# grasingerm/polymer-stats

Hardware: AMD Instinct MI355X
Metric: MC monomer-updates/sec (whole node) at n=100 (higher is better)
Workload: dtype f64

## Files before the change

polymer_stats_amd/csrc/pstat_api.hip:

```cpp
#include <hip/hip_runtime.h>

#include <cmath>
#include <cstdarg>
#include <cstdio>
#include <cstdlib>
#include <cstring>
#include <memory>
#include <new>
#include <vector>

#include "../../include/pstat.h"
#include "pstat_cluster_common.h"
#include "pstat_device.h"

using namespace pstat;

namespace {

thread_local char g_err[512] = "";

int fail(int code, const char *fmt, ...) {
  va_list ap;
  va_start(ap, fmt);
  vsnprintf(g_err, sizeof g_err, fmt, ap);
// ... 357 lines not shown
  p->cutoff_radius = 7.5;
}

int pstat_create(const pstat_params *cases, int32_t ncases, void *stream, pstat_handle **out) {
  if (!cases || !out) return fail(PSTAT_ERR_INVALID_ARG, "null argument");
  *out = nullptr;
  int rc = validate(cases, ncases);
  if (rc) return rc;
  int ndev = pstat_device_count();
  if (ndev < 1) return fail(PSTAT_ERR_NO_DEVICE, "no HIP device is visible (this library has no CPU path)");
  if (cases[0].device < 0 || cases[0].device >= ndev)
    return fail(PSTAT_ERR_NO_DEVICE, "device %d out of range (have %d)", cases[0].device, ndev);

  pstat_handle *h = new (std::nothrow) pstat_handle;
  if (!h) return fail(PSTAT_ERR_NOMEM, "host allocation failed");
  try {
  h->base = cases[0];
  h->ncases = ncases;
  h->device = cases[0].device;
  h->elem = cases[0].precision == PSTAT_F64 ? 8 : (cases[0].precision == PSTAT_Q16 ? 2 : 4);
  for (int i = 0; i < ncases; ++i) {
    const pstat_params &p = cases[i];
    h->cases.push_back({p.E0, p.K1, p.K2, p.mu, p.kT, p.Fz, p.Fx, p.b, p.seed, p.chain_id0,
                        p.bend_mod, p.bend_angle, p.cluster_prob, p.cutoff_radius});
    h->kT0.push_back(p.kT);
  }
  bool any_fx = false;
  for (auto &c : h->cases) any_fx = any_fx || c.Fx != 0.0;
  h->ov = read_overrides();
  h->cfg = {h->base.precision, h->base.chain_type, h->base.energy_type, h->base.do_flips ? 1 : 0,
            h->base.umbrella ? 1 : 0, any_fx ? 1 : 0, 0, h->base.rng, h->base.move_set};
  const Home home = h->cfg.home = choose_home(h->cfg, h->base.n, h->base.num_chains, ncases, h->ov);

  int lanes = (home == SweepLds || home == ClusterLds) ? choose_lanes(h->base.precision, h->base.n, h->base.energy_type) : 64;
  if (lanes == 0) {
    delete h;
    return fail(PSTAT_ERR_UNSUPPORTED, "num-monomers = %lld does not fit the 160 KiB LDS of a CU",
                (long long)cases[0].n);
  }
  SweepArgs &A = h->args;
  A.n = h->base.n;
  A.chains_per_case = h->base.num_chains;
  A.blocks_per_case = (h->base.num_chains + lanes - 1) / lanes;
  A.nblocks = A.blocks_per_case * ncases;
  A.nsteps = 0; A.step0 = 0;
  A.steps_per_adjust = h->base.steps_per_adjust;
  A.adj_lb = h->base.adj_lb; A.adj_ub = h->base.adj_ub; A.adj_scale = h->base.adj_scale;
  A.lanes = lanes;
  A.adaptive = (h->base.adj_scale != 1.0 && h->base.steps_per_adjust > 0) ? 1 : 0;
  A.ncases = ncases; A.seg_len = 0; A.nseg = 1; A.max_spins = 1 << 22;
  A.lds_rows = 0; A.packed = 0; A.pad_ = 0;
  A.wide_eps = (h->base.precision == PSTAT_F64 && h->base.uniform_bits != 23) ? 1 : 0;
  if (home == SweepMem) {
    int rows = 160 * 1024 / 4 / (64 * 16) - 1;
    if (h->ov.f64_lds_rows >= 0 && h->ov.f64_lds_rows <= rows) rows = h->ov.f64_lds_rows;
    A.lds_rows = (int32_t)(h->base.n < rows ? h->base.n : rows);
  }

#define CREATE_TRY(expr)            \
  do {                              \
    int _rc = (expr);               \
    if (_rc) { pstat_destroy(h); return _rc; } \
  } while (0)
#define CREATE_HIP(expr)                                                                   \
  do {                                                                                     \
    hipError_t _e = (expr);                                                                \
    if (_e != hipSuccess) {                                                                \
      pstat_destroy(h);                                                                    \
      return fail(PSTAT_ERR_HIP, "%s failed: %s", #expr, hipGetErrorString(_e));           \
    }                                                                                      \
  } while (0)

  CREATE_HIP(hipSetDevice(h->device));
  hipDeviceProp_t prop;
  if (chain_per_lane(home)) {
    CREATE_HIP(hipGetDeviceProperties(&prop, h->device));
    Shape pick = shape(h->cfg, A, false, false, prop.multiProcessorCount, h->ov.lanes);
    if (ncases > 1) {
      const Shape pk = shape(h->cfg, A, true, pick.cost >= 4.0 || h->ov.pack == 1, prop.multiProcessorCount, h->ov.lanes);
      if (h->ov.pack >= 0 ? h->ov.pack == 1 : pk.cost < 0.95 * pick.cost) {
        pick = pk;
        h->cfg.packed = 1;
        A.packed = 1;
      }
    }
    A.lanes = pick.lanes;
    A.blocks_per_case = (h->base.num_chains + pick.lanes - 1) / pick.lanes;
// ... 526 lines not shown
```

polymer_stats_amd/csrc/pstat_device.h:

```cpp
#pragma once

#include <hip/hip_runtime.h>
#include <stdint.h>

namespace pstat {

enum { OBS_R1 = 0, OBS_R2, OBS_R3, OBS_P1, OBS_P2, OBS_P3, OBS_U, OBS_USUM,
       OBS_C2,
       OBS_PSI,
       NOBS_STATE };
enum { S_R1 = 0, S_R2, S_R3, S_R1SQ, S_R2SQ, S_R3SQ, S_P1, S_P2, S_P3, S_P1SQ, S_P2SQ, S_P3SQ,
       S_U, S_USQ, NSUMS_BASE, S_C2 = NSUMS_BASE, S_PSI, NSUMS };

struct DevState {
  void *ang;
  void *ang_tmp;
  uint32_t *rng;
  double *stepsz;
  int64_t *win;
  int64_t *nacc_total;
  double *obs;
  double *sums;
  double *wnorm;
  double *lag;
// ... 198 lines not shown
struct LaunchCfg {
  int precision, chain_type, energy_type, do_flips, umbrella, has_fx;
  int lag;
  int rng;
  int move_set;
  Home home;
  int packed;
};
hipError_t launch_init(const LaunchCfg &cfg, const SweepArgs &a, const DevState &s,
                       const CaseConst *cases, double phi_step, double theta_step,
                       const InitOpts &io, hipStream_t stream);
hipError_t launch_reset_sampler(const DevState &s, double phi_step, double theta_step, hipStream_t stream);
hipError_t launch_cluster(const LaunchCfg &cfg, const SweepArgs &a, const DevState &s,
                          const CaseConst *cases, int *queue, unsigned grid, hipStream_t stream);
hipError_t cluster_kernel_info(const LaunchCfg &cfg, const SweepArgs &a, int *lds_bytes,
                               int *blocks_per_cu, const char **name);
hipError_t launch_cluster_gm(const LaunchCfg &cfg, const SweepArgs &a, const DevState &s,
                             const CaseConst *cases, int *queue, unsigned grid, hipStream_t stream);
hipError_t cluster_gm_kernel_info(const LaunchCfg &cfg, const SweepArgs &a, int *lds_bytes,
                                  int *blocks_per_cu, const char **name);
size_t cluster_gm_work_bytes(const LaunchCfg &cfg, const SweepArgs &a);
hipError_t launch_sweep(const LaunchCfg &cfg, const SweepArgs &a, const DevState &s,
                        const CaseConst *cases, int *queue, unsigned grid, hipStream_t stream);
size_t sweep_queue_ints(const SweepArgs &a);
hipError_t launch_reinit(const LaunchCfg &cfg, const SweepArgs &a, const DevState &s,
                         const CaseConst *cases, int force_init, hipStream_t stream);
template <typename R> __host__ __device__ inline bool not_finite(R x) { return !__builtin_isfinite(x); }
hipError_t launch_reduce(const DevState &s, int64_t c0, int64_t c1, int64_t steps_recorded,
                         int umbrella, const CaseConst *cases, int64_t chains_per_case, int64_t n,
                         double *partial, double *out, hipStream_t stream);
size_t reduce_scratch_doubles();
hipError_t sweep_kernel_info(const LaunchCfg &cfg, const SweepArgs &a, int *lds_bytes,
                             int *blocks_per_cu, const char **name);
int choose_lanes(int precision, int64_t n, int energy_type);
hipError_t launch_interacting(const LaunchCfg &cfg, const SweepArgs &a, const DevState &s,
                              const CaseConst *cases, int reinit_mode, hipStream_t stream);
hipError_t launch_cluster_wave(const LaunchCfg &cfg, const SweepArgs &a, const DevState &s, const CaseConst *cases,
                               hipStream_t stream);
hipError_t cluster_wave_kernel_info(const LaunchCfg &cfg, int64_t n, int *blocks_per_cu, const char **name);
hipError_t launch_cluster_cw(const LaunchCfg &cfg, const SweepArgs &a, const DevState &s, const CaseConst *cases,
                             hipStream_t stream);
hipError_t cluster_cw_kernel_info(const LaunchCfg &cfg, int64_t n, int *blocks_per_cu, const char **name);
hipError_t interacting_kernel_info(const LaunchCfg &cfg, int64_t n, int *blocks_per_cu, const char **name);

}
```

polymer_stats_amd/csrc/pstat_kernels.hip:

```cpp
#include "pstat_device.h"

#include <hip/hip_runtime.h>
#include <math.h>
#include <type_traits>

#include "../../include/pstat.h"
#include "pstat_math.h"

#ifndef PSTAT_GM_DEPTH
#define PSTAT_GM_DEPTH 2
#endif
#ifndef PSTAT_GI_DEPTH
#define PSTAT_GI_DEPTH 1
#endif
#ifndef PSTAT_GI_CC
#define PSTAT_GI_CC 1
#endif
#ifndef PSTAT_UNROLL_ISING
#define PSTAT_UNROLL_ISING 16
#endif
#ifndef PSTAT_UNROLL
#define PSTAT_UNROLL 16
#endif

// ... 84 lines not shown
  d.w0 = g.next();
  d.idx = __umulhi(d.w0, n);
  d.cell = __umul24(d.idx, row_bytes) + lane_bytes;
  d.wphi = g.next();
  d.wflip = 0;
  if constexpr (RARE) {
    if (flips) d.wflip = g.next();
  }
  d.wth = g.next();
  d.weps = g.next();
  return d;
}

struct SweepRare {
  int flips;
  int lag;
  int umb;
};

template <typename R, typename G, int CT, int EN, bool FX, bool RARE, int ST>
__device__ __forceinline__ void run_segment(const SweepArgs &A, const DevState &S, const CaseConst &cc,
                                            const SweepRare rare, unsigned char *smem, const int lane,
                                            const int64_t c, int64_t step, int64_t remaining, const int blk) {
  using R2 = typename Vec2<R>::type;
  using AG = Ang<R>;
  constexpr bool Q = ST == 1;
  constexpr bool GM = ST == 2;
  static_assert(!Q || sizeof(R) == 4, "the lattice state runs on f32 arithmetic");
  static_assert(!GM || sizeof(R) == 8, "global-memory state: f64");
  constexpr bool GI = GM && EN == PSTAT_ISING;
  constexpr int DEPTH = GI ? PSTAT_GI_DEPTH : PSTAT_GM_DEPTH;
  using Cell = typename std::conditional<Q, uint32_t, R2>::type;
  const int lanes = GM ? 64 : A.lanes;
  unsigned char *const cells = GM ? reinterpret_cast<unsigned char *>(S.work) + (size_t)blk * (size_t)A.n * 64 * sizeof(Cell) : smem;
  Cell *ang = reinterpret_cast<Cell *>(cells);
  const int64_t C = S.C;
  const int n = (int)A.n;

  const R Fz = (R)cc.Fz, Fx = (R)cc.Fx, b = (R)cc.b, kT = (R)cc.kT;
  const R a_or_mu = (CT == PSTAT_DIELECTRIC) ? (R)((cc.K1 - cc.K2) * cc.E0) : (R)cc.mu;
  const R k2e = (R)(cc.K2 * cc.E0);
  const R mhalfE0 = (R)(-0.5 * cc.E0);
  const R hb = (R)(-cc.b / 2);
  const R ising_scale = cc.b == 0.0 ? (R)__builtin_nan("") : (R)(0.0795774715459476679 / fabs(cc.b * cc.b * cc.b / 8));
  const R nbeta_log2e = (R)(-1.4426950408889634 / cc.kT);
  const double ninv_kT = -1.0 / cc.kT;
  (void)ninv_kT;
  (void)Fx; (void)kT; (void)hb; (void)nbeta_log2e; (void)ising_scale;

  R maxphi = 0;
  (void)maxphi;
  if constexpr (Q) {
    const uint16_t *gth = (const uint16_t *)S.ang, *gph = (const uint16_t *)S.ang + (int64_t)n * C;
#pragma unroll 8
    for (int i = 0; i < n; ++i)
      ang[i * lanes + lane] = (uint32_t)gth[(int64_t)i * C + c] | ((uint32_t)gph[(int64_t)i * C + c] << 16);
  } else {
    const R *gth = (const R *)S.ang, *gph = (const R *)S.ang + (int64_t)n * C;
#pragma unroll 8
    for (int i = 0; i < n; ++i) {
      R2 v;
      v.x = gth[(int64_t)i * C + c];
      v.y = gph[(int64_t)i * C + c];
      if constexpr (sizeof(R) == 8) maxphi = fmax(maxphi, fabs(v.y));
      if (GM && i < A.lds_rows) reinterpret_cast<Cell *>(smem)[i * lanes + lane] = v;
      else if constexpr (GM) *reinterpret_cast<Cell *>(cells + ((EN == PSTAT_ISING && PSTAT_GI_CC) ? (uint32_t)lane * (uint32_t)n * (uint32_t)sizeof(Cell) + (uint32_t)i * (uint32_t)sizeof(Cell)
                                                                                                          : (uint32_t)(i * lanes + lane) * (uint32_t)sizeof(Cell))) = v;
      else ang[i * lanes + lane] = v;
    }
  }
  constexpr double th_unit = Q ? 3.14159265358979323846 / 65536.0 : AG::unit;
  constexpr double ph_unit = Q ? 6.28318530717958647692 / 65536.0 : AG::unit;
  G g;
  g.load(S.rng + c, C);
  double phistep_d = S.stepsz[0 * C + c], thstep_d = S.stepsz[1 * C + c];
  R phistep = (R)(phistep_d / ph_unit), thstep = (R)(thstep_d / th_unit);
  int64_t nacc_off = S.win[0 * C + c], natt_off = S.win[1 * C + c];
  int nacc_seg = 0, steps_seg = 0;
  int nnan_seg = 0;
  R O[8];
  O[0] = (R)S.obs[OBS_R1 * C + c]; O[1] = (R)S.obs[OBS_R2 * C + c]; O[2] = (R)S.obs[OBS_R3 * C + c];
  O[3] = (R)S.obs[OBS_P1 * C + c]; O[4] = (R)S.obs[OBS_P2 * C + c]; O[5] = (R)S.obs[OBS_P3 * C + c];
  O[6] = (R)S.obs[OBS_U * C + c]; O[7] = 0;
  R usum = (R)S.obs[OBS_USUM * C + c];
  R lag = RARE ? (R)S.lag[c] : (R)0;
  const bool umb = RARE && rare.umb;
  const R wscale = umb ? (R)((0.2 + 0.8 * exp(-(cc.Fx * cc.Fx + cc.Fz * cc.Fz) / cc.kT)) / cc.kT) : (R)0;
  R uref = umb ? (R)S.uref[c] : (R)0;
  bool regauged = false;
  double wnorm = umb ? S.wnorm[c] : 0.0;
  double sums[NSUMS_BASE];
#pragma unroll
  for (int q = 0; q < NSUMS_BASE; ++q) sums[q] = S.sums[q * C + c];

  const int64_t spa = A.steps_per_adjust;
  int64_t to_adj = A.adaptive ? spa - (step % spa) : 0;
  constexpr int FLUSH = 128;
  const bool flips = RARE && rare.flips;

  using P = typename V2<R>::type;
  const uint32_t row_bytes = (uint32_t)lanes * (uint32_t)sizeof(Cell), lane_bytes = (uint32_t)lane * (uint32_t)sizeof(Cell);
  auto slot = [&](uint32_t off) __attribute__((always_inline)) -> Cell & { return *reinterpret_cast<Cell *>(cells + off); };
  constexpr bool CC = GI && PSTAT_GI_CC;
  const uint32_t chain_g = (uint32_t)lane * (uint32_t)n * (uint32_t)sizeof(Cell);
  auto gofs = [&](const uint32_t idx) __attribute__((always_inline)) -> uint32_t {
    return CC ? chain_g + idx * (uint32_t)sizeof(Cell) : idx * row_bytes + lane_bytes;
  };
  typedef int v4i __attribute__((ext_vector_type(4)));
  struct RowG { Cell l; v4i g; };
  struct RowG3 { RowG c, lo, hi; };
  using Row = typename std::conditional<GI, RowG3, typename std::conditional<GM, RowG, Cell>::type>::type;
  const uint32_t nL = GM ? (uint32_t)A.lds_rows : 0u;
  const uint32_t trash = nL * row_bytes + lane_bytes;
  __amdgpu_buffer_rsrc_t rsrc = __builtin_amdgcn_make_buffer_rsrc(GM ? (void *)cells : (void *)nullptr, 0,
                                                                  GM ? (int)((uint32_t)n * row_bytes) : 0, 0x00020000);
  auto rdcell = [&](const uint32_t idx, const uint32_t cell) __attribute__((always_inline)) -> RowG {
    const bool inL = idx < nL;
    RowG r;
    r.l = *reinterpret_cast<Cell *>(smem + (inL ? cell : trash));
    r.g = __builtin_amdgcn_raw_buffer_load_b128(rsrc, inL ? 0xFFFFFFFFu : gofs(idx), 0, 0);
    return r;
  };
  auto resolve = [&](const RowG &r, const uint32_t idx, const uint32_t cell, const Cell &f1, const uint32_t at1,
                     const Cell &f2, const uint32_t at2, const Cell &f3, const uint32_t at3) __attribute__((always_inline)) -> Cell {
    if constexpr (GM) {
      typedef double v2dd __attribute__((ext_vector_type(2)));
      const v2dd gv = __builtin_bit_cast(v2dd, r.g);
      const bool inL = idx < nL;
      Cell a;
      a.x = inL ? r.l.x : gv.x; a.y = inL ? r.l.y : gv.y;
      if constexpr (DEPTH == 3) {
        const bool s3 = at3 == cell;
        a.x = s3 ? f3.x : a.x; a.y = s3 ? f3.y : a.y;
      }
      if constexpr (DEPTH >= 2) {
        const bool s2 = at2 == cell;
        a.x = s2 ? f2.x : a.x; a.y = s2 ? f2.y : a.y;
      }
      const bool s1 = at1 == cell;
      a.x = s1 ? f1.x : a.x; a.y = s1 ? f1.y : a.y;
      return a;
    } else {
      return r.l;
    }
  };
  auto rdrow = [&](const Draw &d) __attribute__((always_inline)) -> Row {
    if constexpr (GI) {
      const bool hasLo = d.idx > 0, hasHi = d.idx + 1 < (uint32_t)n;
      RowG3 r;
      r.c = rdcell(d.idx, d.cell);
      r.lo = rdcell(hasLo ? d.idx - 1 : d.idx, hasLo ? d.cell - row_bytes : d.cell);
      r.hi = rdcell(hasHi ? d.idx + 1 : d.idx, hasHi ? d.cell + row_bytes : d.cell);
      return r;
    } else if constexpr (GM) {
      return rdcell(d.idx, d.cell);
    } else {
      return slot(d.cell);
    }
  };
  auto wr = [&](const Draw &d, const Cell v, const bool ok) __attribute__((always_inline)) {
    if constexpr (GM) {
      const bool inL = d.idx < nL;
      *reinterpret_cast<Cell *>(smem + ((ok && inL) ? d.cell : trash)) = v;
      typedef double v2dd __attribute__((ext_vector_type(2)));
      const v2dd vv = {v.x, v.y};
      __builtin_amdgcn_raw_buffer_store_b128(__builtin_bit_cast(v4i, vv), rsrc, (ok && !inL) ? gofs(d.idx) : 0xFFFFFFFFu, 0, 0);
    } else {
      slot(d.cell) = v;
    }
  };
  Draw dA = draw_step<RARE>(g, (uint32_t)n, flips, row_bytes, lane_bytes), dB = dA;
  Row aA = rdrow(dA), aB = aA;
  Draw dC = dA;
  Row aC = aA;
  Draw dD = dA;
  Row aD = aA;
  Cell fw1_cell{}, fw2_cell{}, fw3_cell{};
  uint32_t fw1_at = ~0u, fw2_at = ~0u, fw3_at = ~0u;
  (void)dC; (void)aC; (void)dD; (void)aD; (void)fw1_cell; (void)fw2_cell; (void)fw3_cell; (void)fw1_at; (void)fw2_at; (void)fw3_at;
  if constexpr (GM && DEPTH >= 2) {
    if (remaining > 1) {
      dB = draw_step<RARE>(g, (uint32_t)n, flips, row_bytes, lane_bytes);
      aB = rdrow(dB);
    }
    if constexpr (DEPTH == 3) {
      if (remaining > 2) {
        dC = draw_step<RARE>(g, (uint32_t)n, flips, row_bytes, lane_bytes);
        aC = rdrow(dC);
      }
    }
  }
  R phistep3 = 3 * phistep, thstep3 = 3 * thstep;
  (void)phistep3; (void)thstep3;
  P stepv = {thstep, phistep}, step3v = {thstep3, phistep3};
  (void)stepv; (void)step3v;
  int left = (int)remaining;
// ... 80 lines not shown
        if constexpr (RARE) {
          if (flips && (d.wflip >> 31)) k0 = 65535u - k0;
        }
        const int k1 = (int)k0 + q16_disp(thstep, sym11<R>(d.wth));
        const uint32_t j1 = (j0 + (uint32_t)q16_disp(phistep, sym11<R>(d.wphi))) & 0xFFFFu;
        inside = (uint32_t)k1 < 65536u;
        const uint32_t k1c = (uint32_t)min(max(k1, 0), 65535);
        th1 = q16_theta_turns(k1c);
        ph1 = q16_phi_turns(j1);
        cell1 = k1c | (j1 << 16);
      } else {
        th0 = a0.x; ph0 = a0.y;
        R flip = 0;
        if constexpr (RARE) {
          if (flips && (d.wflip >> 31)) flip = AG::theta_max - 2 * th0;
        }
        if constexpr (sizeof(R) == 8) {
          auto rounded = [](R v) __attribute__((always_inline)) -> R { asm volatile("" : "+v"(v)); return v; };
          const R dphi = rounded(phistep * rounded(sym11<R>(d.wphi)));
          R dth = rounded(thstep * rounded(sym11<R>(d.wth)));
          if constexpr (RARE) dth = rounded(flip + dth);
          ph1 = AG::wrap(ph0 + dphi);
          th1 = fmin(AG::theta_max, fmax((R)0, th0 + dth));
        } else {
          R base = th0;
          if constexpr (RARE) base = th0 + flip;
          const P basev = {base, ph0}, fv = {bits24(d.wth), bits24(d.wphi)};
          const P raw = pfma(stepv, fv, basev - step3v);
          th1 = fmin(AG::theta_max, fmax((R)0, raw.x));
          ph1 = AG::wrap(raw.y);
        }
      }
      R st0, ct0, sp0, cp0, st1, ct1, sp1, cp1;
      AG::sc_theta(th0, &st0, &ct0);
      AG::sc_theta(th1, &st1, &ct1);
      AG::template sc_phi<FOLD>(ph0, &sp0, &cp0);
      AG::template sc_phi<FOLD>(ph1, &sp1, &cp1);
      P dNxy, dMxy, D;
      R dpair = 0;
      if constexpr (EN == PSTAT_ISING && sizeof(R) == 4) {
        const P S01 = {st0, st1}, X01 = P{cp0, cp1} * S01, Y01 = P{sp0, sp1} * S01, C01 = {ct0, ct1};
        P MX01, MY01, MZ01;
        if constexpr (CT == PSTAT_DIELECTRIC) {
          const P q01 = C01 * P{a_or_mu, a_or_mu};
          MX01 = q01 * X01; MY01 = q01 * Y01;
          MZ01 = pfma(q01, C01, P{k2e, k2e});
        } else {
          const P mus = {a_or_mu, a_or_mu};
          MX01 = mus * X01; MY01 = mus * Y01; MZ01 = mus * C01;
        }
        dNxy = P{X01.y - X01.x, Y01.y - Y01.x};
        dMxy = P{MX01.y - MX01.x, MY01.y - MY01.x};
        D = P{C01.y - C01.x, MZ01.y - MZ01.x};
        P e01 = {0, 0};
        const P m3 = {-3.0f, -3.0f};
#pragma unroll
        for (int side = -1; side <= 1; side += 2) {
          const int j = (int)d.idx + side;
          if (j >= 0 && j < n) {
            const Cell aj = ang[j * lanes + lane];
            R thj, phj;
            if constexpr (Q) { thj = q16_theta_turns(aj & 0xFFFFu); phj = q16_phi_turns(aj >> 16); }
            else { thj = aj.x; phj = aj.y; }
            R sj, cj, spj, cpj, mjx, mjy, mjz;
            AG::sc(thj, &sj, &cj);
            AG::sc(phj, &spj, &cpj);
            const R njx = cpj * sj, njy = spj * sj, njz = cj;
            dipole<R, CT>(a_or_mu, k2e, njx, njy, njz, mjx, mjy, mjz);
            const P rx = X01 + P{njx, njx}, ry = Y01 + P{njy, njy}, rz = C01 + P{njz, njz};
            const P jx = {mjx, mjx}, jy = {mjy, mjy}, jz = {mjz, mjz};
// ... 5 lines not shown
            const P mjr = pfma(jz, rz, pfma(jy, ry, jx * rx));
            const P num = pfma(m3 * ir2, mir * mjr, mimj);
            e01 = pfma(num, ir2 * ir, e01);
          }
        }
        dpair = (e01.y - e01.x) * ising_scale;
      } else {
        const P cs0 = {cp0, sp0}, cs1 = {cp1, sp1};
        const P s0s = {st0, st0}, s1s = {st1, st1};
        const P Nxy0 = cs0 * s0s, Nxy1 = cs1 * s1s;
        P Mxy0, Mxy1;
        R mz0, mz1;
        if constexpr (CT == PSTAT_DIELECTRIC) {
          const R q0 = a_or_mu * ct0, q1 = a_or_mu * ct1;
          const P q0s = {q0, q0}, q1s = {q1, q1};
          Mxy0 = q0s * Nxy0; Mxy1 = q1s * Nxy1;
          mz0 = q0 * ct0 + k2e; mz1 = q1 * ct1 + k2e;
        } else {
          const P mus = {a_or_mu, a_or_mu};
          Mxy0 = mus * Nxy0; Mxy1 = mus * Nxy1;
          mz0 = a_or_mu * ct0; mz1 = a_or_mu * ct1;
        }
        dNxy = Nxy1 - Nxy0; dMxy = Mxy1 - Mxy0;
        const P Z0 = {ct0, mz0}, Z1 = {ct1, mz1};
        D = Z1 - Z0;

        if constexpr (GI) {
          R e0 = 0, e1 = 0;
#pragma unroll
          for (int side = 0; side < 2; ++side) {
            const Cell aj = side ? aHi : aLo;
            const bool has = side ? d.idx + 1 < (uint32_t)n : d.idx > 0;
            R sj, cj, spj, cpj, mjx, mjy, mjz;
            AG::sc_theta(aj.x, &sj, &cj);
            AG::template sc_phi<FOLD>(aj.y, &spj, &cpj);
            const R njx = cpj * sj, njy = spj * sj, njz = cj;
            dipole<R, CT>(a_or_mu, k2e, njx, njy, njz, mjx, mjy, mjz);
            const R t0 = pair_term_fast(hb * (Nxy0.x + njx), hb * (Nxy0.y + njy), hb * (ct0 + njz),
                                        Mxy0.x, Mxy0.y, mz0, mjx, mjy, mjz);
            const R t1 = pair_term_fast(hb * (Nxy1.x + njx), hb * (Nxy1.y + njy), hb * (ct1 + njz),
                                        Mxy1.x, Mxy1.y, mz1, mjx, mjy, mjz);
            e0 += has ? t0 : (R)0; e1 += has ? t1 : (R)0;
          }
          dpair = e1 - e0;
        } else if constexpr (EN == PSTAT_ISING) {
          R e0 = 0, e1 = 0;
  #pragma unroll
          for (int side = -1; side <= 1; side += 2) {
            const int j = (int)d.idx + side;
            if (j >= 0 && j < n) {
              const Cell aj = ang[j * lanes + lane];
              R thj, phj;
              if constexpr (Q) { thj = q16_theta_turns(aj & 0xFFFFu); phj = q16_phi_turns(aj >> 16); }
              else { thj = aj.x; phj = aj.y; }
              R sj, cj, spj, cpj, mjx, mjy, mjz;
              AG::sc(thj, &sj, &cj);
              AG::sc(phj, &spj, &cpj);
              const R njx = cpj * sj, njy = spj * sj, njz = cj;
              dipole<R, CT>(a_or_mu, k2e, njx, njy, njz, mjx, mjy, mjz);
              e0 += pair_term_fast(hb * (Nxy0.x + njx), hb * (Nxy0.y + njy), hb * (ct0 + njz),
                                   Mxy0.x, Mxy0.y, mz0, mjx, mjy, mjz);
              e1 += pair_term_fast(hb * (Nxy1.x + njx), hb * (Nxy1.y + njy), hb * (ct1 + njz),
                                   Mxy1.x, Mxy1.y, mz1, mjx, mjy, mjz);
            }
          }
          dpair = e1 - e0;
        }
      }
// ... 171 lines not shown
          phistep_d = fmin(K<double>::pi, phistep_d * A.adj_scale);
          thstep_d = fmin(K<double>::half_pi, thstep_d * A.adj_scale);
        } else if (ratio < A.adj_lb) {
          nacc_off = -nacc_seg; natt_off = -steps_seg;
          phistep_d /= A.adj_scale;
          thstep_d /= A.adj_scale;
        }
        phistep = (R)(phistep_d / ph_unit); thstep = (R)(thstep_d / th_unit);
        phistep3 = 3 * phistep; thstep3 = 3 * thstep;
        stepv = P{thstep, phistep}; step3v = P{thstep3, phistep3};
      }
    }
  }
  };
  if constexpr (sizeof(R) == 8) {
    const bool can_reach = !((double)maxphi + 3.1416 * (double)remaining < PSTAT_PHI_FOLD);
    if (__builtin_amdgcn_ballot_w64(can_reach) != 0) run_steps(std::true_type{});
    else run_steps(std::false_type{});
  } else {
    run_steps(std::false_type{});
  }

  if constexpr (Q) {
    uint16_t *gth = (uint16_t *)S.ang, *gph = (uint16_t *)S.ang + (int64_t)n * C;
    for (int i = 0; i < n; ++i) {
      const uint32_t v = ang[i * lanes + lane];
      gth[(int64_t)i * C + c] = (uint16_t)(v & 0xFFFFu);
      gph[(int64_t)i * C + c] = (uint16_t)(v >> 16);
    }
  } else {
    R *gth = (R *)S.ang, *gph = (R *)S.ang + (int64_t)n * C;
    for (int i = 0; i < n; ++i) {
      R2 v;
      if (GM && i < A.lds_rows) v = reinterpret_cast<Cell *>(smem)[i * lanes + lane];
      else if constexpr (GM) v = *reinterpret_cast<Cell *>(cells + gofs((uint32_t)i));
      else v = ang[i * lanes + lane];
      gth[(int64_t)i * C + c] = v.x;
      gph[(int64_t)i * C + c] = v.y;
    }
  }
  g.store(S.rng + c, C);
  S.stepsz[0 * C + c] = phistep_d; S.stepsz[1 * C + c] = thstep_d;
  S.win[0 * C + c] = nacc_off + nacc_seg; S.win[1 * C + c] = natt_off + steps_seg;
  S.nacc_total[c] += nacc_seg;
  if constexpr (EN == PSTAT_ISING) S.nanrej[c] += nnan_seg;
  const R unit_r = sizeof(R) == 4 ? b : (R)1;
  S.obs[OBS_R1 * C + c] = unit_r * Orxy.x; S.obs[OBS_R2 * C + c] = unit_r * Orxy.y; S.obs[OBS_R3 * C + c] = unit_r * Oz.x;
  S.obs[OBS_P1 * C + c] = Opxy.x; S.obs[OBS_P2 * C + c] = Opxy.y; S.obs[OBS_P3 * C + c] = Oz.y;
  S.obs[OBS_U * C + c] = OU;
  if constexpr (RARE) S.obs[OBS_USUM * C + c] = usum;
  if constexpr (RARE) {
    S.lag[c] = lag;
    if (umb) S.wnorm[c] = wnorm;
    if (regauged) S.uref[c] = (double)uref;
  }
#pragma unroll
  for (int q = 0; q < NSUMS_BASE; ++q) S.sums[q * C + c] = sums[q];
}

template <typename R, typename G, int CT, int EN, bool FX, bool RARE, int ST, bool PACKED = false>
__global__ __launch_bounds__(64) void sweep_kernel(SweepArgs A, DevState S,
                                                   const CaseConst *__restrict__ cases,
                                                   SweepRare rare, int *__restrict__ queue) {
  extern __shared__ __attribute__((aligned(16))) unsigned char smem[];
  const int lane = threadIdx.x;
  run_job_queue<PACKED>(A, queue, lane, [&](const CaseConst &cc, int64_t chain, int64_t first, int64_t len, int blk) {
    run_segment<R, G, CT, EN, FX, RARE, ST>(A, S, cc, rare, smem, lane, chain, first, len, blk);
  }, cases);
}

#ifndef PSTAT_PART

constexpr int RED_BLOCKS = 256;
constexpr int RED_THREADS = 256;
constexpr int NQ = 19;
constexpr int NX = 2;
constexpr int NP = 2 * NQ + NX;

__device__ __forceinline__ double wave_sum(double v) {
#pragma unroll
  for (int off = 32; off > 0; off >>= 1) v += __shfl_down(v, off, 64);
  return v;
}

__global__ __launch_bounds__(RED_THREADS) void reduce_stage1(DevState S, int64_t c0, int64_t c1,
                                                             int64_t steps, int umbrella,
                                                             const CaseConst *__restrict__ cases,
                                                             int64_t chains_per_case, int64_t n,
                                                             double *__restrict__ partial) {
  __shared__ double red[RED_THREADS / 64][NP];
  double m1[NQ], m2[NQ], mx[NX] = {0, 0};
#pragma unroll
  for (int q = 0; q < NQ; ++q) { m1[q] = 0; m2[q] = 0; }
  const int64_t C = S.C;
  for (int64_t c = c0 + (int64_t)blockIdx.x * RED_THREADS + threadIdx.x; c < c1;
       c += (int64_t)RED_BLOCKS * RED_THREADS) {
    const double norm = umbrella ? S.wnorm[c] : (double)steps;
    const double inv = norm != 0.0 ? 1.0 / norm : 0.0;
// ... 142 lines not shown
  if (cfg.has_fx) return rare ? pick_state<G, CT, EN, true, true>() : pick_state<G, CT, EN, true, false>();
  return rare ? pick_state<G, CT, EN, false, true>() : pick_state<G, CT, EN, false, false>();
}
template <typename G>
static SweepFn pick_model(const LaunchCfg &cfg) {
  const bool ising = cfg.energy_type == PSTAT_ISING;
  if (cfg.chain_type == PSTAT_DIELECTRIC)
    return ising ? pick_flags<G, PSTAT_DIELECTRIC, PSTAT_ISING>(cfg)
                 : pick_flags<G, PSTAT_DIELECTRIC, PSTAT_NONINTERACTING>(cfg);
  return ising ? pick_flags<G, PSTAT_POLAR, PSTAT_ISING>(cfg)
               : pick_flags<G, PSTAT_POLAR, PSTAT_NONINTERACTING>(cfg);
}
#if PSTAT_PART == 4
SweepFn pick_sweep_f64g(const LaunchCfg &cfg) {
#elif PSTAT_PART == 3
SweepFn pick_sweep_f64(const LaunchCfg &cfg) {
#elif PSTAT_PART == 2
SweepFn pick_sweep_q16(const LaunchCfg &cfg) {
#else
SweepFn pick_sweep_f32(const LaunchCfg &cfg) {
#endif
  return cfg.rng == PSTAT_RNG_XOSHIRO128PP ? pick_model<Xoshiro128pp>(cfg) : pick_model<Mwc64x>(cfg);
}

#else

SweepFn pick_sweep_f32(const LaunchCfg &cfg);
SweepFn pick_sweep_q16(const LaunchCfg &cfg);
SweepFn pick_sweep_f64(const LaunchCfg &cfg);
SweepFn pick_sweep_f64g(const LaunchCfg &cfg);

static int cell_bytes(int precision) { return precision == PSTAT_F64 ? 16 : (precision == PSTAT_Q16 ? 4 : 8); }

int choose_lanes(int precision, int64_t n, int energy_type) {
  (void)energy_type;
  const int64_t per_lane = n * cell_bytes(precision);
  const int64_t budget = 160 * 1024;
  for (int lanes = 64; lanes >= 8; lanes >>= 1)
    if (per_lane * lanes <= budget) return lanes;
  return 0;
}

static SweepFn pick_sweep(const LaunchCfg &cfg) {
  if (cfg.home == SweepMem) return pick_sweep_f64g(cfg);
  return cfg.precision == PSTAT_F64 ? pick_sweep_f64(cfg)
       : (cfg.precision == PSTAT_Q16 ? pick_sweep_q16(cfg) : pick_sweep_f32(cfg));
}

static int sweep_lds_bytes(const LaunchCfg &cfg, const SweepArgs &a) {
  if (cfg.home == SweepMem) return (a.lds_rows + 1) * 64 * 16;
  return (int)(a.n * a.lanes * cell_bytes(cfg.precision));
}

hipError_t sweep_kernel_info(const LaunchCfg &cfg, const SweepArgs &a, int *lds_bytes,
                             int *blocks_per_cu, const char **name) {
  SweepFn fn = pick_sweep(cfg);
  const int lds = sweep_lds_bytes(cfg, a);
  hipError_t e = hipFuncSetAttribute((const void *)fn, hipFuncAttributeMaxDynamicSharedMemorySize, lds);
  if (e != hipSuccess) return e;
  int nb = 0;
  e = hipOccupancyMaxActiveBlocksPerMultiprocessor(&nb, (const void *)fn, 64, lds);
  if (e != hipSuccess) return e;
  if (lds_bytes) *lds_bytes = lds;
  if (blocks_per_cu) *blocks_per_cu = nb;
  if (name) *name = cfg.precision == PSTAT_F64 ? (cfg.home == SweepMem ? (cfg.packed ? "sweep_kernel<double, state in L2> [packed cases]" : "sweep_kernel<double, state in L2>")
                                                                   : (cfg.packed ? "sweep_kernel<double> [packed cases]" : "sweep_kernel<double>"))
                 : (cfg.precision == PSTAT_Q16 ? (cfg.packed ? "sweep_kernel<float, q16 state> [packed cases]" : "sweep_kernel<float, q16 state>")
                                               : (cfg.packed ? "sweep_kernel<float> [packed cases]" : "sweep_kernel<float>"));
  return hipSuccess;
}

size_t sweep_queue_ints(const SweepArgs &a) { return 2 + (size_t)a.nblocks; }

hipError_t launch_sweep(const LaunchCfg &cfg, const SweepArgs &a, const DevState &s,
                        const CaseConst *cases, int *queue, unsigned grid, hipStream_t stream) {
  SweepFn fn = pick_sweep(cfg);
  const int lds = sweep_lds_bytes(cfg, a);
  hipError_t e = hipFuncSetAttribute((const void *)fn, hipFuncAttributeMaxDynamicSharedMemorySize, lds);
  if (e != hipSuccess) return e;
  e = hipMemsetAsync(queue + 1, 0, sizeof(int) * (sweep_queue_ints(a) - 1), stream);
  if (e != hipSuccess) return e;
  SweepRare rare{cfg.do_flips, cfg.lag, cfg.umbrella};
  hipLaunchKernelGGL(fn, dim3(grid), dim3(64), lds, stream, a, s, cases, rare, queue);
  return hipGetLastError();
// ... 71 lines not shown
```

polymer_stats_amd/csrc/pstat_math.h:

```cpp
#pragma once

#include <hip/hip_runtime.h>
#include <math.h>
#include <stdint.h>

#include "../../include/pstat.h"

namespace pstat {


template <typename R> struct Vec2;
template <> struct Vec2<float> { using type = float2; };
template <> struct Vec2<double> { using type = double2; };

template <typename R> struct K;
template <> struct K<double> {
  static constexpr double pi = 3.14159265358979323846;
  static constexpr double half_pi = 1.57079632679489661923;
};

__device__ __forceinline__ double exp_f64(const double x) {
  const double k = rint(x * 1.44269504088896338700e+00);
  const double hi = __builtin_fma(-k, 6.93147180369123816490e-01, x);
  const double r = __builtin_fma(-k, 1.90821492927058770002e-10, hi);
// ... 246 lines not shown
    }
  }
  const double k = rint(x * 6.36619772367581382433e-01);
  const double r = __builtin_fma(-k, 6.12323399573676603587e-17, __builtin_fma(-k, 1.57079632679489655800e+00, x));
  const double z = r * r;
  const double S1 = -1.66666666666666324348e-01, S2 = 8.33333333332248946124e-03, S3 = -1.98412698298579493134e-04,
               S4 = 2.75573137070700676789e-06, S5 = -2.50507602534068634195e-08, S6 = 1.58969099521155010221e-10;
  const double C1 = 4.16666666666666019037e-02, C2 = -1.38888888888741095749e-03, C3 = 2.48015872894767294178e-05,
               C4 = -2.75573143513906633035e-07, C5 = 2.08757232129817482790e-09, C6 = -1.13596475577881948265e-11;
  const double ps = __builtin_fma(z, __builtin_fma(z, __builtin_fma(z, __builtin_fma(z, __builtin_fma(z, S6, S5), S4), S3), S2), S1);
  const double pc = __builtin_fma(z, __builtin_fma(z, __builtin_fma(z, __builtin_fma(z, __builtin_fma(z, C6, C5), C4), C3), C2), C1);
#ifndef PSTAT_THETA_GENERIC_TAIL
  if constexpr (BOUNDED) {
    const double ks = __builtin_fma(r * z, ps, r);
    const double kc = __builtin_fma(z, __builtin_fma(z, pc, -0.5), 1.0);
    const bool one = k == 1.0, two = k == 2.0;
    const double cq = two ? -kc : kc;
    *s = one ? kc : __builtin_fabs(ks);
    *c = one ? -ks : cq;
    return;
  }
#endif
  const uint32_t q = (uint32_t)(int)k;
  const uint32_t odd = q << 31;
  const uint32_t m_kc = (q >> 1) << 31;
  const uint32_t m_ks = m_kc ^ odd;
  const double rs = __hiloint2double((int)(__double2hiint(r) ^ m_ks), __double2loint(r));
  const double ks = __builtin_fma(rs * z, ps, rs);
  const double kc0 = __builtin_fma(z, __builtin_fma(z, pc, -0.5), 1.0);
  const double kc = __hiloint2double((int)(__double2hiint(kc0) ^ m_kc), __double2loint(kc0));
  const bool swap = (int)odd < 0;
  *s = swap ? kc : ks;
  *c = swap ? ks : kc;
}

__device__ __forceinline__ float acos_r(float x) {
  const float a = fabsf(x);
  float p = -0.0012624911f;
  p = __builtin_fmaf(p, a, 0.0066700901f);
  p = __builtin_fmaf(p, a, -0.0170881256f);
  p = __builtin_fmaf(p, a, 0.0308918810f);
  p = __builtin_fmaf(p, a, -0.0501743046f);
  p = __builtin_fmaf(p, a, 0.0889789874f);
  p = __builtin_fmaf(p, a, -0.2145988016f);
  p = __builtin_fmaf(p, a, 1.5707963050f);
  const float r = __builtin_amdgcn_sqrtf(fmaxf(1.0f - a, 0.0f)) * p;
  return x < 0.0f ? 3.14159265358979f - r : r;
}
__device__ __forceinline__ double acos_r(double x) {
  const double a = fabs(x);
  const bool big = a >= 0.5;
  const double z = big ? __builtin_fma(a, -0.5, 0.5) : a * a;
  double p = 2.87578513674215663354e-02;
  p = __builtin_fma(p, z, -1.48518870712472036977e-02);
  p = __builtin_fma(p, z, 1.74008794426940213707e-02);
  p = __builtin_fma(p, z, 5.45750671864035814818e-03);
  p = __builtin_fma(p, z, 1.03228143501857792808e-02);
  p = __builtin_fma(p, z, 1.14791774151849056834e-02);
  p = __builtin_fma(p, z, 1.39712129735529329289e-02);
  p = __builtin_fma(p, z, 1.73523927208699725588e-02);
  p = __builtin_fma(p, z, 2.23721729421498885526e-02);
  p = __builtin_fma(p, z, 3.03819441385312465076e-02);
  p = __builtin_fma(p, z, 4.46428571463554288434e-02);
  p = __builtin_fma(p, z, 7.49999999999843292020e-02);
  p = __builtin_fma(p, z, 1.66666666666666685170e-01);
  const double zp = z * p;
  const double y = __builtin_amdgcn_rsq(z);
  const double s0 = z * y, h0 = 0.5 * y;
  const double r = __builtin_fma(-s0, h0, 0.5);
  const double s1 = __builtin_fma(s0, r, s0), h1 = __builtin_fma(h0, r, h0);
  double sq = __builtin_fma(__builtin_fma(-s1, s1, z), h1, s1);
  sq = z == 0.0 ? 0.0 : sq;
  const double t = big ? sq : x;
  const double as = __builtin_fma(t, zp, t);
  const double small = 1.57079632679489661923 - as;
  const double two = as + as;
  const double bigv = x < 0.0 ? 3.14159265358979323846 - two : two;
  return big ? bigv : small;
}

template <typename R> struct Ang;
template <> struct Ang<double> {
  static constexpr double theta_max = 3.14159265358979323846;
  static constexpr double unit = 1.0;
  static __device__ __forceinline__ void sc(double x, double *s, double *c) { sincos_f64(x, s, c); }
  static __device__ __forceinline__ void sc_theta(double x, double *s, double *c) { sincos_fast_f64<true>(x, s, c); }
  template <bool FOLD = true>
  static __device__ __forceinline__ void sc_phi(double x, double *s, double *c) { sincos_fast_f64<false, FOLD>(x, s, c); }
  static __device__ __forceinline__ double wrap(double x) { return x; }
};
template <> struct Ang<float> {
  static constexpr float theta_max = 0.5f;
  static constexpr double unit = 6.28318530717958647692;
  static __device__ __forceinline__ void sc(float x, float *s, float *c) {
    *s = __builtin_amdgcn_sinf(x);
    *c = __builtin_amdgcn_cosf(x);
  }
  static __device__ __forceinline__ void sc_theta(float x, float *s, float *c) { sc(x, s, c); }
  template <bool FOLD = true>
  static __device__ __forceinline__ void sc_phi(float x, float *s, float *c) { sc(x, s, c); }
  static __device__ __forceinline__ float wrap(float x) { return __builtin_amdgcn_fractf(x); }
};


}
```

Before: 102.8 billion.

## Use LDS-resident 64-entry sincos table for f64 angle evaluation in sweep kernel

Replaces the polynomial f64 sincos in the sweep kernel with a table-driven scheme. The argument is reduced to a multiple of pi/32 plus a small remainder, the sin/cos of the multiple is looked up from a 1 KiB table held in LDS, and a short polynomial on the remainder finishes the result. The kernel fills the table at startup, and the LDS budgets (lanes, rows) are shrunk to make room for it. The aim is to cut FP64 instruction count per proposal, at the cost of extra LDS reads, possible bank conflicts, slightly less LDS for cells, and different rounding behaviour.

```diff
diff --git a/polymer_stats_amd/csrc/pstat_api.hip b/polymer_stats_amd/csrc/pstat_api.hip
--- a/polymer_stats_amd/csrc/pstat_api.hip
+++ b/polymer_stats_amd/csrc/pstat_api.hip
@@ -413,7 +413,8 @@
             h->base.umbrella ? 1 : 0, any_fx ? 1 : 0, 0, h->base.rng, h->base.move_set};
   const Home home = h->cfg.home = choose_home(h->cfg, h->base.n, h->base.num_chains, ncases, h->ov);
 
-  int lanes = (home == SweepLds || home == ClusterLds) ? choose_lanes(h->base.precision, h->base.n, h->base.energy_type) : 64;
+  const int tab_bytes = (home == SweepLds && h->base.precision == PSTAT_F64) ? PSTAT_SINCOS_TAB_BYTES : 0;
+  int lanes = (home == SweepLds || home == ClusterLds) ? choose_lanes(h->base.precision, h->base.n, h->base.energy_type, tab_bytes) : 64;
   if (lanes == 0) {
     delete h;
     return fail(PSTAT_ERR_UNSUPPORTED, "num-monomers = %lld does not fit the 160 KiB LDS of a CU",
@@ -433,7 +434,7 @@
   A.lds_rows = 0; A.packed = 0; A.pad_ = 0;
   A.wide_eps = (h->base.precision == PSTAT_F64 && h->base.uniform_bits != 23) ? 1 : 0;
   if (home == SweepMem) {
-    int rows = 160 * 1024 / 4 / (64 * 16) - 1;
+    int rows = 160 * 1024 / 4 / (64 * 16) - 2;
     if (h->ov.f64_lds_rows >= 0 && h->ov.f64_lds_rows <= rows) rows = h->ov.f64_lds_rows;
     A.lds_rows = (int32_t)(h->base.n < rows ? h->base.n : rows);
   }
diff --git a/polymer_stats_amd/csrc/pstat_device.h b/polymer_stats_amd/csrc/pstat_device.h
--- a/polymer_stats_amd/csrc/pstat_device.h
+++ b/polymer_stats_amd/csrc/pstat_device.h
@@ -254,7 +254,8 @@
 size_t reduce_scratch_doubles();
 hipError_t sweep_kernel_info(const LaunchCfg &cfg, const SweepArgs &a, int *lds_bytes,
                              int *blocks_per_cu, const char **name);
-int choose_lanes(int precision, int64_t n, int energy_type);
+#define PSTAT_SINCOS_TAB_BYTES 1024
+int choose_lanes(int precision, int64_t n, int energy_type, int table_bytes);
 hipError_t launch_interacting(const LaunchCfg &cfg, const SweepArgs &a, const DevState &s,
                               const CaseConst *cases, int reinit_mode, hipStream_t stream);
 hipError_t launch_cluster_wave(const LaunchCfg &cfg, const SweepArgs &a, const DevState &s, const CaseConst *cases,
diff --git a/polymer_stats_amd/csrc/pstat_kernels.hip b/polymer_stats_amd/csrc/pstat_kernels.hip
--- a/polymer_stats_amd/csrc/pstat_kernels.hip
+++ b/polymer_stats_amd/csrc/pstat_kernels.hip
@@ -140,7 +140,10 @@
   constexpr int DEPTH = GI ? PSTAT_GI_DEPTH : PSTAT_GM_DEPTH;
   using Cell = typename std::conditional<Q, uint32_t, R2>::type;
   const int lanes = GM ? 64 : A.lanes;
-  unsigned char *const cells = GM ? reinterpret_cast<unsigned char *>(S.work) + (size_t)blk * (size_t)A.n * 64 * sizeof(Cell) : smem;
+  const unsigned char *const tab = smem;
+  unsigned char *const lds = smem + (sizeof(R) == 8 ? PSTAT_SINCOS_TAB_BYTES : 0);
+  (void)tab;
+  unsigned char *const cells = GM ? reinterpret_cast<unsigned char *>(S.work) + (size_t)blk * (size_t)A.n * 64 * sizeof(Cell) : lds;
   Cell *ang = reinterpret_cast<Cell *>(cells);
   const int64_t C = S.C;
   const int n = (int)A.n;
@@ -171,7 +174,7 @@
       v.x = gth[(int64_t)i * C + c];
       v.y = gph[(int64_t)i * C + c];
       if constexpr (sizeof(R) == 8) maxphi = fmax(maxphi, fabs(v.y));
-      if (GM && i < A.lds_rows) reinterpret_cast<Cell *>(smem)[i * lanes + lane] = v;
+      if (GM && i < A.lds_rows) reinterpret_cast<Cell *>(lds)[i * lanes + lane] = v;
       else if constexpr (GM) *reinterpret_cast<Cell *>(cells + ((EN == PSTAT_ISING && PSTAT_GI_CC) ? (uint32_t)lane * (uint32_t)n * (uint32_t)sizeof(Cell) + (uint32_t)i * (uint32_t)sizeof(Cell)
                                                                                                           : (uint32_t)(i * lanes + lane) * (uint32_t)sizeof(Cell))) = v;
       else ang[i * lanes + lane] = v;
@@ -225,7 +228,7 @@
   auto rdcell = [&](const uint32_t idx, const uint32_t cell) __attribute__((always_inline)) -> RowG {
     const bool inL = idx < nL;
     RowG r;
-    r.l = *reinterpret_cast<Cell *>(smem + (inL ? cell : trash));
+    r.l = *reinterpret_cast<Cell *>(lds + (inL ? cell : trash));
     r.g = __builtin_amdgcn_raw_buffer_load_b128(rsrc, inL ? 0xFFFFFFFFu : gofs(idx), 0, 0);
     return r;
   };
@@ -269,7 +272,7 @@
   auto wr = [&](const Draw &d, const Cell v, const bool ok) __attribute__((always_inline)) {
     if constexpr (GM) {
       const bool inL = d.idx < nL;
-      *reinterpret_cast<Cell *>(smem + ((ok && inL) ? d.cell : trash)) = v;
+      *reinterpret_cast<Cell *>(lds + ((ok && inL) ? d.cell : trash)) = v;
       typedef double v2dd __attribute__((ext_vector_type(2)));
       const v2dd vv = {v.x, v.y};
       __builtin_amdgcn_raw_buffer_store_b128(__builtin_bit_cast(v4i, vv), rsrc, (ok && !inL) ? gofs(d.idx) : 0xFFFFFFFFu, 0, 0);
@@ -416,10 +419,21 @@
         }
       }
       R st0, ct0, sp0, cp0, st1, ct1, sp1, cp1;
-      AG::sc_theta(th0, &st0, &ct0);
-      AG::sc_theta(th1, &st1, &ct1);
-      AG::template sc_phi<FOLD>(ph0, &sp0, &cp0);
-      AG::template sc_phi<FOLD>(ph1, &sp1, &cp1);
+      if constexpr (sizeof(R) == 8) {
+        const SincosArg r0 = sincos_tab_reduce<false>(th0), r1 = sincos_tab_reduce<false>(th1);
+        const SincosArg r2 = sincos_tab_reduce<FOLD>(ph0), r3 = sincos_tab_reduce<FOLD>(ph1);
+        const double2 e0 = *reinterpret_cast<const double2 *>(tab + r0.at), e1 = *reinterpret_cast<const double2 *>(tab + r1.at);
+        const double2 e2 = *reinterpret_cast<const double2 *>(tab + r2.at), e3 = *reinterpret_cast<const double2 *>(tab + r3.at);
+        sincos_tab_finish(r0.r, e0, &st0, &ct0);
+        sincos_tab_finish(r1.r, e1, &st1, &ct1);
+        sincos_tab_finish(r2.r, e2, &sp0, &cp0);
+        sincos_tab_finish(r3.r, e3, &sp1, &cp1);
+      } else {
+        AG::sc_theta(th0, &st0, &ct0);
+        AG::sc_theta(th1, &st1, &ct1);
+        AG::template sc_phi<FOLD>(ph0, &sp0, &cp0);
+        AG::template sc_phi<FOLD>(ph1, &sp1, &cp1);
+      }
       P dNxy, dMxy, D;
       R dpair = 0;
       if constexpr (EN == PSTAT_ISING && sizeof(R) == 4) {
@@ -491,8 +505,8 @@
             const Cell aj = side ? aHi : aLo;
             const bool has = side ? d.idx + 1 < (uint32_t)n : d.idx > 0;
             R sj, cj, spj, cpj, mjx, mjy, mjz;
-            AG::sc_theta(aj.x, &sj, &cj);
-            AG::template sc_phi<FOLD>(aj.y, &spj, &cpj);
+            AG::sc_theta(aj.x, tab, &sj, &cj);
+            AG::template sc_phi<FOLD>(aj.y, tab, &spj, &cpj);
             const R njx = cpj * sj, njy = spj * sj, njz = cj;
             dipole<R, CT>(a_or_mu, k2e, njx, njy, njz, mjx, mjy, mjz);
             const R t0 = pair_term_fast(hb * (Nxy0.x + njx), hb * (Nxy0.y + njy), hb * (ct0 + njz),
@@ -730,7 +744,7 @@
     R *gth = (R *)S.ang, *gph = (R *)S.ang + (int64_t)n * C;
     for (int i = 0; i < n; ++i) {
       R2 v;
-      if (GM && i < A.lds_rows) v = reinterpret_cast<Cell *>(smem)[i * lanes + lane];
+      if (GM && i < A.lds_rows) v = reinterpret_cast<Cell *>(lds)[i * lanes + lane];
       else if constexpr (GM) v = *reinterpret_cast<Cell *>(cells + gofs((uint32_t)i));
       else v = ang[i * lanes + lane];
       gth[(int64_t)i * C + c] = v.x;
@@ -762,6 +776,10 @@
                                                    SweepRare rare, int *__restrict__ queue) {
   extern __shared__ __attribute__((aligned(16))) unsigned char smem[];
   const int lane = threadIdx.x;
+  if constexpr (sizeof(R) == 8) {
+    fill_sincos_tab(smem, lane);
+    __syncthreads();
+  }
   run_job_queue<PACKED>(A, queue, lane, [&](const CaseConst &cc, int64_t chain, int64_t first, int64_t len, int blk) {
     run_segment<R, G, CT, EN, FX, RARE, ST>(A, S, cc, rare, smem, lane, chain, first, len, blk);
   }, cases);
@@ -970,10 +988,10 @@
 
 static int cell_bytes(int precision) { return precision == PSTAT_F64 ? 16 : (precision == PSTAT_Q16 ? 4 : 8); }
 
-int choose_lanes(int precision, int64_t n, int energy_type) {
+int choose_lanes(int precision, int64_t n, int energy_type, int table_bytes) {
   (void)energy_type;
   const int64_t per_lane = n * cell_bytes(precision);
-  const int64_t budget = 160 * 1024;
+  const int64_t budget = 160 * 1024 - table_bytes;
   for (int lanes = 64; lanes >= 8; lanes >>= 1)
     if (per_lane * lanes <= budget) return lanes;
   return 0;
@@ -986,8 +1004,9 @@
 }
 
 static int sweep_lds_bytes(const LaunchCfg &cfg, const SweepArgs &a) {
-  if (cfg.home == SweepMem) return (a.lds_rows + 1) * 64 * 16;
-  return (int)(a.n * a.lanes * cell_bytes(cfg.precision));
+  const int tab = cfg.precision == PSTAT_F64 ? PSTAT_SINCOS_TAB_BYTES : 0;
+  if (cfg.home == SweepMem) return (a.lds_rows + 1) * 64 * 16 + tab;
+  return (int)(a.n * a.lanes * cell_bytes(cfg.precision)) + tab;
 }
 
 hipError_t sweep_kernel_info(const LaunchCfg &cfg, const SweepArgs &a, int *lds_bytes,
diff --git a/polymer_stats_amd/csrc/pstat_math.h b/polymer_stats_amd/csrc/pstat_math.h
--- a/polymer_stats_amd/csrc/pstat_math.h
+++ b/polymer_stats_amd/csrc/pstat_math.h
@@ -302,6 +302,108 @@
   const bool swap = (int)odd < 0;
   *s = swap ? kc : ks;
   *c = swap ? ks : kc;
+}
+
+static __constant__ const double sincos_tab_pi32[64][2] = {
+    {0x0.0p+0, 0x1.0000000000000p+0},
+    {0x1.917a6bc29b42cp-4, 0x1.fd88da3d12526p-1},
+    {0x1.8f8b83c69a60bp-3, 0x1.f6297cff75cb0p-1},
+    {0x1.294062ed59f06p-2, 0x1.e9f4156c62ddap-1},
+    {0x1.87de2a6aea963p-2, 0x1.d906bcf328d46p-1},
+    {0x1.e2b5d3806f63bp-2, 0x1.c38b2f180bdb1p-1},
+    {0x1.1c73b39ae68c8p-1, 0x1.a9b66290ea1a3p-1},
+    {0x1.44cf325091dd6p-1, 0x1.8bc806b151741p-1},
+    {0x1.6a09e667f3bcdp-1, 0x1.6a09e667f3bcdp-1},
+    {0x1.8bc806b151741p-1, 0x1.44cf325091dd6p-1},
+    {0x1.a9b66290ea1a3p-1, 0x1.1c73b39ae68c8p-1},
+    {0x1.c38b2f180bdb1p-1, 0x1.e2b5d3806f63bp-2},
+    {0x1.d906bcf328d46p-1, 0x1.87de2a6aea963p-2},
+    {0x1.e9f4156c62ddap-1, 0x1.294062ed59f06p-2},
+    {0x1.f6297cff75cb0p-1, 0x1.8f8b83c69a60bp-3},
+    {0x1.fd88da3d12526p-1, 0x1.917a6bc29b42cp-4},
+    {0x1.0000000000000p+0, 0x0.0p+0},
+    {0x1.fd88da3d12526p-1, -0x1.917a6bc29b42cp-4},
+    {0x1.f6297cff75cb0p-1, -0x1.8f8b83c69a60bp-3},
+    {0x1.e9f4156c62ddap-1, -0x1.294062ed59f06p-2},
+    {0x1.d906bcf328d46p-1, -0x1.87de2a6aea963p-2},
+    {0x1.c38b2f180bdb1p-1, -0x1.e2b5d3806f63bp-2},
+    {0x1.a9b66290ea1a3p-1, -0x1.1c73b39ae68c8p-1},
+    {0x1.8bc806b151741p-1, -0x1.44cf325091dd6p-1},
+    {0x1.6a09e667f3bcdp-1, -0x1.6a09e667f3bcdp-1},
+    {0x1.44cf325091dd6p-1, -0x1.8bc806b151741p-1},
+    {0x1.1c73b39ae68c8p-1, -0x1.a9b66290ea1a3p-1},
+    {0x1.e2b5d3806f63bp-2, -0x1.c38b2f180bdb1p-1},
+    {0x1.87de2a6aea963p-2, -0x1.d906bcf328d46p-1},
+    {0x1.294062ed59f06p-2, -0x1.e9f4156c62ddap-1},
+    {0x1.8f8b83c69a60bp-3, -0x1.f6297cff75cb0p-1},
+    {0x1.917a6bc29b42cp-4, -0x1.fd88da3d12526p-1},
+    {0x0.0p+0, -0x1.0000000000000p+0},
+    {-0x1.917a6bc29b42cp-4, -0x1.fd88da3d12526p-1},
+    {-0x1.8f8b83c69a60bp-3, -0x1.f6297cff75cb0p-1},
+    {-0x1.294062ed59f06p-2, -0x1.e9f4156c62ddap-1},
+    {-0x1.87de2a6aea963p-2, -0x1.d906bcf328d46p-1},
+    {-0x1.e2b5d3806f63bp-2, -0x1.c38b2f180bdb1p-1},
+    {-0x1.1c73b39ae68c8p-1, -0x1.a9b66290ea1a3p-1},
+    {-0x1.44cf325091dd6p-1, -0x1.8bc806b151741p-1},
+    {-0x1.6a09e667f3bcdp-1, -0x1.6a09e667f3bcdp-1},
+    {-0x1.8bc806b151741p-1, -0x1.44cf325091dd6p-1},
+    {-0x1.a9b66290ea1a3p-1, -0x1.1c73b39ae68c8p-1},
+    {-0x1.c38b2f180bdb1p-1, -0x1.e2b5d3806f63bp-2},
+    {-0x1.d906bcf328d46p-1, -0x1.87de2a6aea963p-2},
+    {-0x1.e9f4156c62ddap-1, -0x1.294062ed59f06p-2},
+    {-0x1.f6297cff75cb0p-1, -0x1.8f8b83c69a60bp-3},
+    {-0x1.fd88da3d12526p-1, -0x1.917a6bc29b42cp-4},
+    {-0x1.0000000000000p+0, 0x0.0p+0},
+    {-0x1.fd88da3d12526p-1, 0x1.917a6bc29b42cp-4},
+    {-0x1.f6297cff75cb0p-1, 0x1.8f8b83c69a60bp-3},
+    {-0x1.e9f4156c62ddap-1, 0x1.294062ed59f06p-2},
+    {-0x1.d906bcf328d46p-1, 0x1.87de2a6aea963p-2},
+    {-0x1.c38b2f180bdb1p-1, 0x1.e2b5d3806f63bp-2},
+    {-0x1.a9b66290ea1a3p-1, 0x1.1c73b39ae68c8p-1},
+    {-0x1.8bc806b151741p-1, 0x1.44cf325091dd6p-1},
+    {-0x1.6a09e667f3bcdp-1, 0x1.6a09e667f3bcdp-1},
+    {-0x1.44cf325091dd6p-1, 0x1.8bc806b151741p-1},
+    {-0x1.1c73b39ae68c8p-1, 0x1.a9b66290ea1a3p-1},
+    {-0x1.e2b5d3806f63bp-2, 0x1.c38b2f180bdb1p-1},
+    {-0x1.87de2a6aea963p-2, 0x1.d906bcf328d46p-1},
+    {-0x1.294062ed59f06p-2, 0x1.e9f4156c62ddap-1},
+    {-0x1.8f8b83c69a60bp-3, 0x1.f6297cff75cb0p-1},
+    {-0x1.917a6bc29b42cp-4, 0x1.fd88da3d12526p-1},
+};
+static_assert(sizeof(sincos_tab_pi32) == 1024, "one 16-byte entry per lane of a wave (PSTAT_SINCOS_TAB_BYTES, pstat_device.h)");
+__device__ __forceinline__ void fill_sincos_tab(unsigned char *lds, const int lane) {
+  const double2 v = {sincos_tab_pi32[lane & 63][0], sincos_tab_pi32[lane & 63][1]};
+  reinterpret_cast<double2 *>(lds)[lane & 63] = v;
+}
+struct SincosArg { double k, r; uint32_t at; };
+template <bool FOLD>
+__device__ __forceinline__ SincosArg sincos_tab_reduce(double x) {
+  if constexpr (FOLD) {
+    if (!(fabs(x) < PSTAT_PHI_FOLD)) {
+      const double t = rint(x * 1.59154943091895345609e-01);
+      x = __builtin_fma(-t, 2.44929359829470641435e-16, __builtin_fma(-t, 6.28318530717958623200e+00, x));
+    }
+  }
+  SincosArg a;
+  const double t = __builtin_fma(x, 0x1.45f306dc9c883p+3, 0x1.8p52);
+  a.k = t - 0x1.8p52;
+  a.r = __builtin_fma(-a.k, 0x1.1a62633145c07p-58, __builtin_fma(-a.k, 0x1.921fb54442d18p-4, x));
+  a.at = ((uint32_t)__double2loint(t) & 63u) * 16u;
+  return a;
+}
+__device__ __forceinline__ void sincos_tab_finish(const double r, const double2 e, double *s, double *c) {
+  const double z = r * r;
+  const double sr = __builtin_fma(r * z, __builtin_fma(z, __builtin_fma(z, -0x1.a013217697587p-13, 0x1.111111072b683p-7),
+                                                       -0x1.5555555555451p-3), r);
+  const double cm1 = z * __builtin_fma(z, __builtin_fma(z, __builtin_fma(z, 0x1.a013d3a5ee6ecp-16, -0x1.6c16c1619af17p-10),
+                                                        0x1.55555555554a4p-5), -0.5);
+  *s = e.x + __builtin_fma(e.y, sr, e.x * cm1);
+  *c = e.y + __builtin_fma(e.y, cm1, -(e.x * sr));
+}
+template <bool FOLD>
+__device__ __forceinline__ void sincos_tab_f64(const double x, const unsigned char *tab, double *s, double *c) {
+  const SincosArg a = sincos_tab_reduce<FOLD>(x);
+  sincos_tab_finish(a.r, *reinterpret_cast<const double2 *>(tab + a.at), s, c);
 }
 
 __device__ __forceinline__ float acos_r(float x) {
@@ -357,6 +459,9 @@
   static __device__ __forceinline__ void sc_theta(double x, double *s, double *c) { sincos_fast_f64<true>(x, s, c); }
   template <bool FOLD = true>
   static __device__ __forceinline__ void sc_phi(double x, double *s, double *c) { sincos_fast_f64<false, FOLD>(x, s, c); }
+  static __device__ __forceinline__ void sc_theta(double x, const unsigned char *tab, double *s, double *c) { sincos_tab_f64<false>(x, tab, s, c); }
+  template <bool FOLD = true>
+  static __device__ __forceinline__ void sc_phi(double x, const unsigned char *tab, double *s, double *c) { sincos_tab_f64<FOLD>(x, tab, s, c); }
   static __device__ __forceinline__ double wrap(double x) { return x; }
 };
 template <> struct Ang<float> {
@@ -369,6 +474,9 @@
   static __device__ __forceinline__ void sc_theta(float x, float *s, float *c) { sc(x, s, c); }
   template <bool FOLD = true>
   static __device__ __forceinline__ void sc_phi(float x, float *s, float *c) { sc(x, s, c); }
+  static __device__ __forceinline__ void sc_theta(float x, const unsigned char *, float *s, float *c) { sc(x, s, c); }
+  template <bool FOLD = true>
+  static __device__ __forceinline__ void sc_phi(float x, const unsigned char *, float *s, float *c) { sc(x, s, c); }
   static __device__ __forceinline__ float wrap(float x) { return __builtin_amdgcn_fractf(x); }
 };
 
```

Result: slower. 101.1 billion (median of 2 runs) (-1.7%).
